# davidbau/rewriting

Hardware: AMD Instinct MI355X
Metric: images/sec StyleGANv2-1024 fwd (higher is better)
Workload: dtype f32 (conv operands split into exact f16 pairs from 32x32 up, f32 accumulate); 1 GPU; stylegan2-1024 generator forward (FFHQ-1024 architecture); batch_per_gpu=64, mconv=seq, weights=synthetic seed 0, parallelism=seeds partitioned per rank, no collective, matrix_mode=split, direct_sums=auto

## Files before the change

### include/rewriting_hip.h

```cpp
#ifndef REWRITING_HIP_H
#define REWRITING_HIP_H

#include <stdint.h>

#ifdef __cplusplus
extern "C" {
#endif

typedef void* rw_stream_t;

#define RW_ERR_BAD_ARGUMENT 10001
#define RW_ERR_UNSUPPORTED  10002

int rw_abi_version(void);
const char* rw_error_string(int code);


int rw_fused_bias_act_f32(const float* x, const float* b, const float* ref, float* y,
                          int64_t n, int64_t step_b, int64_t size_b,
                          int act, int grad, float alpha, float scale, rw_stream_t stream);
int rw_fused_bias_act_f16(const uint16_t* x, const uint16_t* b, const uint16_t* ref, uint16_t* y,
                          int64_t n, int64_t step_b, int64_t size_b,
                          int act, int grad, float alpha, float scale, rw_stream_t stream);
int rw_fused_bias_act_f64(const double* x, const double* b, const double* ref, double* y,
// ... 132 lines not shown
int rw_conv3x3_wino4h_to_rgb_f32(const float* x, const float* uf, int batch, int in_ch, int out_ch, int h, int w,
                                 float w_scale, const rw_conv_epilogue* ep, const rw_rgb_epilogue* rgb, float u_inv,
                                 const float* x_amax, rw_stream_t stream);
long long rw_packed_conv_transpose_blur_wino4h_elems(int out_ch, int in_ch);
int rw_pack_conv_transpose_blur_weight_wino4h_f32(const float* w, const float* k4, float* uf, int out_ch, int in_ch,
                                                  float u_scale, rw_stream_t stream);
int rw_conv_transpose3x3s2_blur_wino4h_f32(const float* x, const float* uf, float* y, int batch, int in_ch,
                                           int out_ch, int h, int w, float w_scale, const rw_conv_epilogue* ep,
                                           const float* post_scale, float u_inv, const float* x_amax,
                                           float* y_amax, rw_stream_t stream);

int rw_dconv3x3_supported(int out_ch, int in_ch, int h, int w);
long long rw_packed_dconv_weight_elems(int out_ch, int in_ch);
int rw_pack_dconv_weight_f32(const float* w, float* wp, int out_ch, int in_ch, float u_scale, rw_stream_t stream);
int rw_dconv3x3_f32(const float* x, const float* wp, float* y, int batch, int in_ch, int out_ch, int h, int w,
                    float w_scale, const rw_conv_epilogue* ep, float u_inv, const float* x_amax, float* y_amax,
                    rw_stream_t stream);
int rw_dconv3x3_rgb_partials(int out_ch);
int rw_dconv3x3_rgb_partial_f32(const float* x, const float* wp, float* y, int batch, int in_ch, int out_ch, int h, int w,
                                float w_scale, const rw_conv_epilogue* ep, const rw_rgb_epilogue* rgb, float u_inv,
                                const float* x_amax, float* y_amax, rw_stream_t stream);
int rw_rgb_combine_f32(const float* partials, int n_part, const float* bias, const float* skip, float* y, int batch,
                       int64_t hw, rw_stream_t stream);
int rw_dconv3x3_to_rgb_supported(int out_ch, int in_ch, int h, int w);
int rw_dconv3x3_to_rgb_f32(const float* x, const float* wp, int batch, int in_ch, int out_ch, int h, int w,
                           float w_scale, const rw_conv_epilogue* ep, const rw_rgb_epilogue* rgb, float u_inv,
                           const float* x_amax, rw_stream_t stream);
int rw_dconv_transpose_blur_supported(int out_ch, int in_ch, int h, int w);
long long rw_packed_dconv_transpose_blur_weight_elems(int out_ch, int in_ch);
int rw_pack_dconv_transpose_blur_weight_f32(const float* w, const float* k4, float* wp, int out_ch, int in_ch,
                                            float u_scale, rw_stream_t stream);
int rw_dconv_transpose3x3s2_blur_f32(const float* x, const float* wp, float* y, int batch, int in_ch, int out_ch, int h,
                                     int w, float w_scale, const rw_conv_epilogue* ep, const float* post_scale,
                                     float u_inv, const float* x_amax, float* y_amax, rw_stream_t stream);

int rw_tconv_blur_supported(int out_ch, int in_ch, int h, int w);
int rw_tconv_blur_f32(const float* x, const float* wp, const float* k4, float* y, int batch, int in_ch, int out_ch, int h,
                      int w, float w_scale, const rw_conv_epilogue* ep, const float* post_scale, float u_inv,
                      const float* x_amax, float* y_amax, rw_stream_t stream);

int rw_conv_transpose3x3s2_winoh_supported(int out_ch, int in_ch, int h, int w);
long long rw_packed_conv_transpose_winoh_elems(int out_ch, int in_ch);
int rw_pack_conv_transpose_winoh_f32(const float* w, float* uf, int out_ch, int in_ch, float u_scale, rw_stream_t stream);
int rw_conv_transpose3x3s2_winoh_f32(const float* x, const float* uf, float* y, int batch, int in_ch, int out_ch,
                                     int h, int w, float w_scale, const float* style, const float* demod, float u_inv,
                                     const float* x_amax, rw_stream_t stream);

int rw_noise_add_f32(const float* x, const float* noise, const float* noise_w, float* y,
                     int batch, int channels, int64_t hw, rw_stream_t stream);

int rw_blur_noise_act_f32(const float* x, const float* k4, const float* noise, const float* noise_w,
                          const float* bias, float* y, int batch, int channels, int out_h, int out_w,
                          rw_stream_t stream);
int rw_blur_noise_act_scaled_f32(const float* x, const float* k4, const float* noise, const float* noise_w,
                                 const float* bias, const float* post_scale, float* y, int batch, int channels,
                                 int out_h, int out_w, rw_stream_t stream);
int rw_blur_noise_act_amax_f32(const float* x, const float* k4, const float* noise, const float* noise_w,
                               const float* bias, const float* post_scale, float* y, int batch, int channels,
                               int out_h, int out_w, float* y_amax, rw_stream_t stream);

int rw_to_rgb_f32(const float* x, const float* w, const float* style, const float* bias,
                  const float* skip, float* y, int batch, int in_ch, int64_t hw, float w_scale,
                  rw_stream_t stream);


int64_t rw_second_moment_workspace_bytes(int channels, int64_t rows);
int rw_second_moment_f32(const float* a, float* mom2, int64_t rows, int channels, int64_t hw,
                         int layout, void* workspace, rw_stream_t stream);

int rw_channel_sums_f32(const float* a, float* sums, int64_t rows, int channels, int64_t hw,
                        int layout, int square_input, rw_stream_t stream);

#define RW_KEY_RESPONSE_MAX_KEYS 8
int rw_key_response_f32(const float* a, const float* keys, float* heat, float* peak,
                        int64_t images, int channels, int64_t hw, int n_keys, rw_stream_t stream);


typedef struct rw_solve_problem {
  int out_ch, in_ch, h, w, rank;
  const float* key;
  const float* style;
  const float* val;
  const float* bias;
  const float* noise;
  const float* noise_w;
  const float* context;
// ... 84 lines not shown
```

### rewriting_amd/_lib.py

```python
import ctypes
import os
from ctypes import (POINTER, Structure, c_char_p, c_double, c_float, c_int, c_int32, c_int64, c_uint,
                    c_void_p)

_HERE = os.path.dirname(os.path.abspath(__file__))
LIB_PATH = os.environ.get('RW_HIP_LIB') or os.path.join(_HERE, 'librewriting_hip.so')

ABI_VERSION = 10


class ConvEpilogue(Structure):
    _fields_ = [('style', c_void_p), ('demod', c_void_p), ('noise', c_void_p),
                ('noise_w', c_void_p), ('bias', c_void_p), ('act', c_int)]


class RgbEpilogue(Structure):
    _fields_ = [('weight', c_void_p), ('style', c_void_p), ('bias', c_void_p), ('skip', c_void_p),
                ('out', c_void_p), ('scale', c_float)]


class SolveProblem(Structure):
    _fields_ = [
        ('out_ch', c_int), ('in_ch', c_int), ('h', c_int), ('w', c_int), ('rank', c_int),
        ('key', c_void_p), ('style', c_void_p), ('val', c_void_p), ('bias', c_void_p),
# ... 93 lines not shown
    'rw_dconv_transpose_blur_weight_absmax_f32': (c_int, [c_void_p, c_void_p, c_int, c_int, c_void_p, c_void_p]),
    'rw_packed_conv_weight_wino4h_elems': (ctypes.c_longlong, [c_int, c_int]),
    'rw_pack_conv_weight_wino4h_f32': (c_int, [c_void_p, c_void_p, c_int, c_int, c_float, c_void_p]),
    'rw_conv3x3_wino4h_f32': (c_int, [c_void_p, c_void_p, c_void_p, c_int, c_int, c_int, c_int, c_int, c_float,
                                      POINTER(ConvEpilogue), c_float, c_void_p, c_void_p, c_void_p]),
    'rw_conv3x3_wino4h_to_rgb_f32': (c_int, [c_void_p, c_void_p, c_int, c_int, c_int, c_int, c_int, c_float,
                                             POINTER(ConvEpilogue), POINTER(RgbEpilogue), c_float, c_void_p, c_void_p]),
    'rw_packed_conv_transpose_blur_wino4h_elems': (ctypes.c_longlong, [c_int, c_int]),
    'rw_pack_conv_transpose_blur_weight_wino4h_f32': (c_int, [c_void_p, c_void_p, c_void_p, c_int, c_int, c_float,
                                                              c_void_p]),
    'rw_conv_transpose3x3s2_blur_wino4h_f32': (c_int, [c_void_p, c_void_p, c_void_p, c_int, c_int, c_int, c_int,
                                                       c_int, c_float, POINTER(ConvEpilogue), c_void_p, c_float,
                                                       c_void_p, c_void_p, c_void_p]),
    'rw_dconv3x3_supported': (c_int, [c_int, c_int, c_int, c_int]),
    'rw_packed_dconv_weight_elems': (ctypes.c_longlong, [c_int, c_int]),
    'rw_pack_dconv_weight_f32': (c_int, [c_void_p, c_void_p, c_int, c_int, c_float, c_void_p]),
    'rw_dconv3x3_f32': (c_int, [c_void_p, c_void_p, c_void_p, c_int, c_int, c_int, c_int, c_int, c_float,
                                POINTER(ConvEpilogue), c_float, c_void_p, c_void_p, c_void_p]),
    'rw_dconv3x3_rgb_partials': (c_int, [c_int]),
    'rw_dconv3x3_rgb_partial_f32': (c_int, [c_void_p, c_void_p, c_void_p, c_int, c_int, c_int, c_int, c_int, c_float,
                                            POINTER(ConvEpilogue), POINTER(RgbEpilogue), c_float, c_void_p, c_void_p,
                                            c_void_p]),
    'rw_rgb_combine_f32': (c_int, [c_void_p, c_int, c_void_p, c_void_p, c_void_p, c_int, c_int64, c_void_p]),
    'rw_dconv3x3_to_rgb_supported': (c_int, [c_int, c_int, c_int, c_int]),
    'rw_dconv3x3_to_rgb_f32': (c_int, [c_void_p, c_void_p, c_int, c_int, c_int, c_int, c_int, c_float,
                                       POINTER(ConvEpilogue), POINTER(RgbEpilogue), c_float, c_void_p, c_void_p]),
    'rw_dconv_transpose_blur_supported': (c_int, [c_int, c_int, c_int, c_int]),
    'rw_packed_dconv_transpose_blur_weight_elems': (ctypes.c_longlong, [c_int, c_int]),
    'rw_pack_dconv_transpose_blur_weight_f32': (c_int, [c_void_p, c_void_p, c_void_p, c_int, c_int, c_float, c_void_p]),
    'rw_dconv_transpose3x3s2_blur_f32': (c_int, [c_void_p, c_void_p, c_void_p, c_int, c_int, c_int, c_int, c_int,
                                                 c_float, POINTER(ConvEpilogue), c_void_p, c_float, c_void_p, c_void_p,
                                                 c_void_p]),
    'rw_tconv_blur_supported': (c_int, [c_int, c_int, c_int, c_int]),
    'rw_tconv_blur_f32': (c_int, [c_void_p, c_void_p, c_void_p, c_void_p, c_int, c_int, c_int, c_int, c_int, c_float,
                                  POINTER(ConvEpilogue), c_void_p, c_float, c_void_p, c_void_p, c_void_p]),
    'rw_conv_transpose_blur_wino4_supported': (c_int, [c_int, c_int, c_int, c_int]),
    'rw_packed_conv_transpose_blur_wino4_elems': (ctypes.c_longlong, [c_int, c_int]),
    'rw_pack_conv_transpose_blur_weight_wino4_f32': (c_int, [c_void_p, c_void_p, c_void_p, c_int, c_int, c_void_p]),
    'rw_conv_transpose3x3s2_blur_wino4_f32': (c_int, [c_void_p, c_void_p, c_void_p, c_int, c_int, c_int, c_int,
                                                      c_int, c_float, POINTER(ConvEpilogue), c_void_p, c_void_p]),
    'rw_blur_noise_act_scaled_f32': (c_int, [c_void_p, c_void_p, c_void_p, c_void_p, c_void_p, c_void_p, c_void_p,
                                             c_int, c_int, c_int, c_int, c_void_p]),
    'rw_blur_noise_act_amax_f32': (c_int, [c_void_p, c_void_p, c_void_p, c_void_p, c_void_p, c_void_p, c_void_p,
                                           c_int, c_int, c_int, c_int, c_void_p, c_void_p]),
    'rw_solve_ksplit': (c_int, [c_int, c_int, c_int, c_int]),
    'rw_solve_supported': (c_int, [c_int] * 7),
# ... 71 lines not shown
```

### rewriting_amd/csrc/rw_common.h

```cpp
#pragma once
#include <hip/hip_runtime.h>
#include <stdint.h>
#include <stdlib.h>
#include "../../include/rewriting_hip.h"

#define RW_WAVE 64

#define RW_CHECK_ARG(cond) do { if (!(cond)) return RW_ERR_BAD_ARGUMENT; } while (0)
#define RW_LAUNCH_RESULT() ((int)hipGetLastError())

static inline hipStream_t rw_s(rw_stream_t s) { return (hipStream_t)s; }

static inline int64_t rw_cdiv(int64_t a, int64_t b) { return (a + b - 1) / b; }

static inline int rw_cu_count(void) {
  static int cached[64];
  int dev = 0;
  if (hipGetDevice(&dev) != hipSuccess || dev < 0 || dev >= 64) return 256;
  if (cached[dev] == 0) {
    int n = 0;
    cached[dev] = (hipDeviceGetAttribute(&n, hipDeviceAttributeMultiprocessorCount, dev) == hipSuccess && n > 0) ? n : 256;
  }
  return cached[dev];
}
// ... 16 lines not shown
  for (int off = 32; off > 0; off >>= 1) v = fmaxf(v, __shfl_xor(v, off, 64));
  return v;
}

__device__ __forceinline__ float rw_block_sum_256(float v, float* lds4) {
  v = rw_wave_sum(v);
  const int wave = threadIdx.x >> 6;
  __syncthreads();
  if ((threadIdx.x & 63) == 0) lds4[wave] = v;
  __syncthreads();
  return lds4[0] + lds4[1] + lds4[2] + lds4[3];
}

typedef float rw_f32x16 __attribute__((ext_vector_type(16)));
typedef float rw_f32x4 __attribute__((ext_vector_type(4)));
typedef float rw_f32x2 __attribute__((ext_vector_type(2)));
typedef unsigned rw_u32x2 __attribute__((ext_vector_type(2)));
typedef unsigned rw_u32x4 __attribute__((ext_vector_type(4)));
typedef int rw_i32x4 __attribute__((ext_vector_type(4)));
typedef _Float16 rw_f16x2 __attribute__((ext_vector_type(2)));
typedef _Float16 rw_f16x4 __attribute__((ext_vector_type(4)));
typedef _Float16 rw_f16x8 __attribute__((ext_vector_type(8)));

template <int N> struct rw_int { static constexpr int value = N; };

__device__ __forceinline__ int rw_xcd_remap(int id, int total) {
  const int q = total >> 3, r = total & 7;
  const int xcd = id & 7, slot = id >> 3;
  const int base = (xcd < r) ? xcd * (q + 1) : r * (q + 1) + (xcd - r) * q;
  return base + slot;
}

__device__ __forceinline__ int rw_swz(int cc) { return (cc >> 1) & 3; }
__device__ __forceinline__ rw_f16x8 rw_expand(rw_f32x2 w) {
  const rw_f32x4 d = {w[0], w[1], w[0], w[1]};
  return __builtin_bit_cast(rw_f16x8, d);
}
__device__ __forceinline__ rw_f16x8 rw_pair(rw_f16x8 a, rw_f16x8 b) {
  return rw_f16x8{a[0], a[1], a[2], a[3], b[0], b[1], b[2], b[3]};
}
__device__ __forceinline__ rw_f16x8 rw_pair(rw_f32x2 a, rw_f32x2 b) {
  const rw_f32x4 d = {a[0], a[1], b[0], b[1]};
  return __builtin_bit_cast(rw_f16x8, d);
}

__device__ __forceinline__ void rw_dma_buffer_b32(unsigned lds_addr, int voffset, rw_i32x4 rsrc, int soffset) {
// ... 76 lines not shown
```

### rewriting_amd/csrc/rw_ops.hip

```cpp
#include "rw_common.h"
#ifndef OPS_NTS
#define OPS_NTS 0
#endif
#include <stdlib.h>
#include <stdint.h>

extern "C" int rw_abi_version(void) { return 10; }

extern "C" const char* rw_error_string(int code) {
  if (code == 0) return "success";
  if (code == RW_ERR_BAD_ARGUMENT) return "rewriting_hip: bad argument";
  if (code == RW_ERR_UNSUPPORTED) return "rewriting_hip: unsupported configuration";
  return hipGetErrorString((hipError_t)code);
}

template <typename T> struct RwAcc { typedef T type; };
template <> struct RwAcc<_Float16> { typedef float type; };

template <typename A>
__device__ __forceinline__ A rw_bias_act_one(A x, A ref, int code, A alpha, A scale) {
  A y;
  switch (code) {
    default:
    case 10: y = x; break;
// ... 957 lines not shown
    return rw_absmax_f32(y, (long long)n_out, y_amax, stream);
  }
  hipLaunchKernelGGL(blur_noise_act_kernel, dim3((unsigned)blocks), dim3(256), 0, rw_s(stream), x, k4,
                     noise, noise_w, bias, y, batch, channels, out_h, out_w, tiles_x, tiles_y, post_scale, y_amax);
  const int rc = RW_LAUNCH_RESULT();
  if (rc || !y_amax) return rc;
  return rw_bound_finish(y_amax, blocks, rw_s(stream));
}

extern "C" int rw_blur_noise_act_scaled_f32(const float* x, const float* k4, const float* noise,
                                            const float* noise_w, const float* bias, const float* post_scale,
                                            float* y, int batch, int channels, int out_h, int out_w,
                                            rw_stream_t stream) {
  return rw_blur_noise_act_amax_f32(x, k4, noise, noise_w, bias, post_scale, y, batch, channels, out_h, out_w, nullptr,
                                    stream);
}

extern "C" int rw_blur_noise_act_f32(const float* x, const float* k4, const float* noise,
                                     const float* noise_w, const float* bias, float* y, int batch,
                                     int channels, int out_h, int out_w, rw_stream_t stream) {
  return rw_blur_noise_act_scaled_f32(x, k4, noise, noise_w, bias, nullptr, y, batch, channels, out_h, out_w, stream);
}

__global__ void __launch_bounds__(256) to_rgb_kernel(const float* __restrict__ x,
                                                     const float* __restrict__ w,
                                                     const float* __restrict__ style,
                                                     const float* __restrict__ bias,
                                                     const float* __restrict__ skip,
                                                     float* __restrict__ y, int in_ch, int64_t hw,
                                                     float w_scale) {
  extern __shared__ float wm[];
  const int b = blockIdx.y;
  for (int t = threadIdx.x; t < 3 * in_ch; t += 256) {
    const int i = t % in_ch;
    wm[t] = w_scale * w[t] * style[(int64_t)b * in_ch + i];
  }
  __syncthreads();
  const int64_t hw4 = hw >> 2;
  const float* xb = x + (int64_t)b * in_ch * hw;
  for (int64_t q = (int64_t)blockIdx.x * 256 + threadIdx.x; q < hw4; q += (int64_t)gridDim.x * 256) {
    float4 a0 = make_float4(0.f, 0.f, 0.f, 0.f), a1 = a0, a2 = a0;
#pragma unroll 8
    for (int i = 0; i < in_ch; ++i) {
      const float4 v = reinterpret_cast<const float4*>(xb + (int64_t)i * hw)[q];
      const float w0 = wm[i], w1 = wm[in_ch + i], w2 = wm[2 * in_ch + i];
      a0.x += w0 * v.x; a0.y += w0 * v.y; a0.z += w0 * v.z; a0.w += w0 * v.w;
      a1.x += w1 * v.x; a1.y += w1 * v.y; a1.z += w1 * v.z; a1.w += w1 * v.w;
      a2.x += w2 * v.x; a2.y += w2 * v.y; a2.z += w2 * v.z; a2.w += w2 * v.w;
    }
    float4 acc[3] = {a0, a1, a2};
#pragma unroll
    for (int c = 0; c < 3; ++c) {
      const float bv = bias ? bias[c] : 0.f;
      float4 o = acc[c];
      o.x += bv; o.y += bv; o.z += bv; o.w += bv;
      const int64_t off = ((int64_t)b * 3 + c) * hw4 + q;
      if (skip) {
        const float4 s = reinterpret_cast<const float4*>(skip)[off];
        o.x += s.x; o.y += s.y; o.z += s.z; o.w += s.w;
      }
#if OPS_NTS & 2
      __builtin_nontemporal_store(rw_f32x4{o.x, o.y, o.z, o.w}, reinterpret_cast<rw_f32x4*>(y) + off);
#else
      reinterpret_cast<float4*>(y)[off] = o;
#endif
    }
  }
}

__global__ void __launch_bounds__(256) rgb_combine_kernel(const float* __restrict__ part, int n_part,
                                                          const float* __restrict__ bias, const float* __restrict__ skip,
                                                          float* __restrict__ y, int64_t n4, int64_t hw4, int64_t stride4) {
  for (int64_t q = (int64_t)blockIdx.x * 256 + threadIdx.x; q < n4; q += (int64_t)gridDim.x * 256) {
    float4 a = reinterpret_cast<const float4*>(part)[q];
    for (int k = 1; k < n_part; ++k) {
      const float4 v = reinterpret_cast<const float4*>(part)[q + k * stride4];
      a.x += v.x; a.y += v.y; a.z += v.z; a.w += v.w;
    }
    if (bias) {
      const float bv = bias[(q / hw4) % 3];
      a.x += bv; a.y += bv; a.z += bv; a.w += bv;
    }
    if (skip) {
      const float4 s = reinterpret_cast<const float4*>(skip)[q];
      a.x += s.x; a.y += s.y; a.z += s.z; a.w += s.w;
    }
    reinterpret_cast<float4*>(y)[q] = a;
  }
}

extern "C" int rw_rgb_combine_f32(const float* partials, int n_part, const float* bias, const float* skip, float* y,
                                  int batch, int64_t hw, rw_stream_t stream) {
  RW_CHECK_ARG(partials && y && n_part > 0 && batch > 0 && hw > 0);
  if (hw % 4) return RW_ERR_UNSUPPORTED;
  const int64_t n4 = (int64_t)batch * 3 * hw / 4;
  hipLaunchKernelGGL(rgb_combine_kernel, dim3(rw_stream_grid(n4, 256)), dim3(256), 0, rw_s(stream), partials, n_part, bias,
                     skip, y, n4, hw / 4, n4);
  return RW_LAUNCH_RESULT();
}

__global__ void __launch_bounds__(256) to_rgb_scalar_kernel(const float* __restrict__ x, const float* __restrict__ w,
                                                            const float* __restrict__ style,
                                                            const float* __restrict__ bias,
                                                            const float* __restrict__ skip, float* __restrict__ y,
                                                            int in_ch, int64_t hw, float w_scale) {
  extern __shared__ float wm[];
  const int b = blockIdx.y;
  for (int t = threadIdx.x; t < 3 * in_ch; t += 256) wm[t] = w_scale * w[t] * style[(int64_t)b * in_ch + t % in_ch];
  __syncthreads();
  const float* xb = x + (int64_t)b * in_ch * hw;
  for (int64_t q = (int64_t)blockIdx.x * 256 + threadIdx.x; q < hw; q += (int64_t)gridDim.x * 256) {
    float a[3] = {0.f, 0.f, 0.f};
    for (int i = 0; i < in_ch; ++i) {
      const float v = xb[(int64_t)i * hw + q];
      a[0] += wm[i] * v; a[1] += wm[in_ch + i] * v; a[2] += wm[2 * in_ch + i] * v;
    }
#pragma unroll
    for (int c = 0; c < 3; ++c) {
      const int64_t off = ((int64_t)b * 3 + c) * hw + q;
      float o = a[c] + (bias ? bias[c] : 0.f);
// ... 2 lines not shown
    }
  }
}

extern "C" int rw_to_rgb_f32(const float* x, const float* w, const float* style, const float* bias,
                             const float* skip, float* y, int batch, int in_ch, int64_t hw,
                             float w_scale, rw_stream_t stream) {
  RW_CHECK_ARG(x && w && style && y && batch > 0 && in_ch > 0 && hw > 0);
  if (hw % 4) {
    int gs = (int)rw_cdiv(hw, 256);
    if (gs > 2048) gs = 2048;
    hipLaunchKernelGGL(to_rgb_scalar_kernel, dim3(gs, batch), dim3(256), 3 * in_ch * sizeof(float), rw_s(stream), x, w,
                       style, bias, skip, y, in_ch, hw, w_scale);
    return RW_LAUNCH_RESULT();
  }
  int gx = (int)rw_cdiv(hw / 4, 256);
  const int cap = (256 * 8 + batch - 1) / batch;
  if (gx > cap) gx = cap;
  if (gx < 1) gx = 1;
  hipLaunchKernelGGL(to_rgb_kernel, dim3(gx, batch), dim3(256), 3 * in_ch * sizeof(float),
                     rw_s(stream), x, w, style, bias, skip, y, in_ch, hw, w_scale);
  return RW_LAUNCH_RESULT();
}
```

### rewriting_amd/hip.py

```python
import ctypes

import torch

from . import _lib
from ._lib import ConvEpilogue, RgbEpilogue, SolveProblem, check

SQRT2 = 2 ** 0.5


def _stream():
    return ctypes.c_void_p(torch.cuda.current_stream().cuda_stream)


def _dev(t, name='tensor', dtype=torch.float32):
    if not isinstance(t, torch.Tensor):
        raise TypeError('%s must be a torch.Tensor' % name)
    if not t.is_cuda:
        raise RuntimeError('rewriting_amd: %s is on %s; the HIP kernels need a GPU tensor '
                           '(there is no CPU fallback)' % (name, t.device))
    if t.dtype != dtype:
        if dtype == torch.float32:
            raise RuntimeError('rewriting_amd: %s is %s; the C ABI is fp32 only (RW_ERR_UNSUPPORTED, include/rewriting_hip.h: '
                               'the reference\'s pybind modules also dispatch half and double, this library does not) -- '
                               'cast the model / tensor with .float()' % (name, t.dtype))
# ... 163 lines not shown
def pack_conv_weight(weight, mode):
    weight = _dev(weight, 'weight')
    o, i = weight.shape[-4], weight.shape[-3]
    n = lib().rw_packed_conv_weight_elems(o, i, int(mode))
    if n <= 0:
        raise ValueError('bad weight shape / mode')
    wp = torch.empty(n, device=weight.device, dtype=weight.dtype)
    check(lib().rw_pack_conv_weight_f32(_p(weight), _p(wp), o, i, int(mode), _stream()))
    return wp


def _check_packed(wp, out_ch, in_ch, mode):
    if wp.numel() != lib().rw_packed_conv_weight_elems(out_ch, in_ch, mode):
        raise ValueError('packed weight does not come from pack_conv_weight(%d x %d, mode %d)'
                         % (out_ch, in_ch, mode))


def _epilogue(style=None, demod=None, noise=None, noise_w=None, bias=None, act=False):
    keep = [_opt(style, 'style'), _opt(demod, 'demod'), _opt(noise, 'noise'),
            _opt(noise_w, 'noise weight'), _opt(bias, 'bias')]
    ep = ConvEpilogue(_p(keep[0]).value, _p(keep[1]).value, _p(keep[2]).value,
                      _p(keep[3]).value, _p(keep[4]).value, int(bool(act)))
    return ep, keep


def _rgb_epilogue(rgb_weight, rgb_style, rgb_bias, rgb_skip, rgb_scale, out, x, out_ch):
    keep = [_dev(rgb_weight, 'rgb weight'), _dev(rgb_style, 'rgb style'), _opt(rgb_bias, 'rgb bias'),
            _opt(rgb_skip, 'rgb skip'), out]
    b, _, h, w = x.shape
    if tuple(keep[0].shape) != (3, out_ch) or tuple(keep[1].shape) != (b, out_ch):
        raise ValueError('rgb weight / style shapes')
    if keep[3] is not None and tuple(keep[3].shape) != (b, 3, h, w):
        raise ValueError('rgb skip shape')
    return RgbEpilogue(*[_p(t).value for t in keep], float(rgb_scale)), keep


def _packed(t, out_ch, in_ch, what, plain=None, split=None):
    wp = _dev(t, 'packed weight')
    if plain is not None and wp.numel() == plain(out_ch, in_ch):
        return wp, None
    if split is not None and wp.numel() == split(out_ch, in_ch):
        return wp, _u_inv(t)
    raise ValueError('packed weight does not come from %s(%d x %d)' % (what, out_ch, in_ch))


def _k4(k4):
# ... 376 lines not shown


def conv3x3_direct16_rgb_partial(x, wp, out_ch, w_scale, rgb_weight, rgb_style, rgb_scale, style=None, demod=None, noise=None,
                                 noise_w=None, bias=None, act=False, x_amax=None, y_amax=None):
    x = _dev(x, 'fmap')
    b, i, h, w = x.shape
    n_part = lib().rw_dconv3x3_rgb_partials(out_ch)
    if n_part <= 0:
        raise ValueError('no ToRGB partial sums for %d out-channels' % out_ch)
    part = torch.empty(n_part, b, 3, h, w, device=x.device, dtype=x.dtype)
    re, rgb_keep = _rgb_epilogue(rgb_weight, rgb_style, None, None, rgb_scale, part, x, out_ch)
    wp, u_inv = _packed(wp, out_ch, i, 'pack_conv_weight_direct16', split=lib().rw_packed_dconv_weight_elems)
    y = torch.empty(b, out_ch, h, w, device=x.device, dtype=x.dtype)
    ep, keep = _epilogue(style, demod, noise, noise_w, bias, act)
    x_amax, y_amax = _amax_in(x, x_amax), _amax_out(y_amax, y.numel())
    check(lib().rw_dconv3x3_rgb_partial_f32(_p(x), _p(wp), _p(y), b, i, out_ch, h, w, float(w_scale), ctypes.byref(ep),
                                            ctypes.byref(re), u_inv, _p(x_amax), _p(y_amax), _stream()))
    return y, part


def rgb_combine(partials, bias, skip):
    partials = _dev(partials, 'rgb partial sums')
    bias = _opt(bias, 'rgb bias')
    skip = _opt(skip, 'rgb skip')
    n, b, c, h, w = partials.shape
    if c != 3 or (skip is not None and tuple(skip.shape) != (b, 3, h, w)):
        raise ValueError('rgb partial / skip shapes')
    y = torch.empty(b, 3, h, w, device=partials.device, dtype=partials.dtype)
    check(lib().rw_rgb_combine_f32(_p(partials), n, _p(bias), _p(skip), _p(y), b, h * w, _stream()))
    return y


def conv3x3_direct16_to_rgb(x, wp, out_ch, w_scale, rgb_weight, rgb_style, rgb_bias, rgb_skip, rgb_scale, style=None,
                            demod=None, noise=None, noise_w=None, bias=None, act=False, x_amax=None):
    x = _dev(x, 'fmap')
    b, i, h, w = x.shape
    rgb = torch.empty(b, 3, h, w, device=x.device, dtype=x.dtype)
    re, rgb_keep = _rgb_epilogue(rgb_weight, rgb_style, rgb_bias, rgb_skip, rgb_scale, rgb, x, out_ch)
    wp, u_inv = _packed(wp, out_ch, i, 'pack_conv_weight_direct16', split=lib().rw_packed_dconv_weight_elems)
    ep, keep = _epilogue(style, demod, noise, noise_w, bias, act)
    x_amax = _amax_in(x, x_amax)
    check(lib().rw_dconv3x3_to_rgb_f32(_p(x), _p(wp), b, i, out_ch, h, w, float(w_scale), ctypes.byref(ep),
                                       ctypes.byref(re), u_inv, _p(x_amax), _stream()))
    return None, rgb


def pack_conv_transpose_blur_weight_direct16(weight, k4):
    weight = _dev(weight, 'weight')
    k4 = _k4(k4)
    o, i = weight.shape[-4], weight.shape[-3]
    n = lib().rw_packed_dconv_transpose_blur_weight_elems(o, i)
# ... 49 lines not shown
    return y


def blur_noise_act(x, k4, noise, noise_w, bias, post_scale=None, y_amax=None):
    x = _dev(x, 'fmap')
    k4 = _dev(k4, 'blur kernel')
    noise = _opt(noise, 'noise')
    noise_w = _opt(noise_w, 'noise weight')
    bias = _opt(bias, 'bias')
    b, c, ih, iw = x.shape
    y = torch.empty(b, c, ih - 1, iw - 1, device=x.device, dtype=x.dtype)
    post_scale = _post_scale(post_scale, b, c, 'channels')
    y_amax = _amax_out(y_amax, y.numel())
    check(lib().rw_blur_noise_act_amax_f32(_p(x), _p(k4), _p(noise), _p(noise_w), _p(bias), _p(post_scale), _p(y),
                                           b, c, ih - 1, iw - 1, _p(y_amax), _stream()))
    return y


def to_rgb(x, weight, style, bias, skip, w_scale):
    x = _dev(x, 'fmap')
    weight = _dev(weight, 'rgb weight')
    style = _dev(style, 'style')
    bias = _opt(bias, 'bias')
    skip = _opt(skip, 'skip')
    b, c, h, w = x.shape
    y = torch.empty(b, 3, h, w, device=x.device, dtype=x.dtype)
    check(lib().rw_to_rgb_f32(_p(x), _p(weight), _p(style), _p(bias), _p(skip), _p(y), b, c, h * w,
                              float(w_scale), _stream()))
    return y


_workspaces = {}


def _workspace(nbytes, device):
    key = (device.index, 'ws')
    ws = _workspaces.get(key)
    if ws is None or ws.numel() < nbytes:
        ws = torch.empty(max(nbytes, 1 << 20), dtype=torch.uint8, device=device)
        _workspaces[key] = ws
    return ws


def second_moment_accumulate(mom2, a, nchw=False):
    a = _dev(a, 'sample')
    if not (mom2.is_cuda and mom2.dtype == torch.float32 and mom2.is_contiguous()):
        raise RuntimeError('mom2 must be a contiguous float32 GPU tensor')
    if nchw:
        b, c, h, w = a.shape
# ... 296 lines not shown
```

### rewriting_amd/utils/stylegan2/models.py

```python
import contextlib
import math
import re
import threading
import warnings
from collections import OrderedDict, namedtuple

import numpy as np
import torch
from torch import nn

from . import grad, op, routing
from .routing import switches
from ... import hip


_weight_epoch = [0]


def bump_weight_epoch():
    _weight_epoch[0] += 1


class _DerivedWeights:

# ... 76 lines not shown
        if t is not None and t.dtype != x.dtype:
            raise RuntimeError('rewriting_amd: %s: the input is %s and the %s %s -- cast the model and its input to one '
                               'dtype, .float() or .double() (nothing is converted)' % (what, x.dtype, name, t.dtype))
    return True


def _forward_only_f64(what, *tensors):
    if torch.is_grad_enabled() and any(t is not None and t.requires_grad for t in tensors):
        raise NotImplementedError('rewriting_amd: %s: the float64 path is forward only -- no graph is recorded for double '
                                  'tensors (the adjoints in utils/stylegan2/grad.py are float32); run it under '
                                  'torch.no_grad(), or differentiate a .float() model' % what)


def _unhooked(*modules):
    return all('forward' not in m.__dict__ for m in modules)


def _idle():
    return dict(
        stream=None,
        aux=None,
        keep=[],
        final=None,
        image_path=False,
        switches=None,
        neighbours={},
        pre={},
        pre_join=None)


class _RunningForward(threading.local):
    def __init__(self):
        vars(self).update(_idle())


_running = _RunningForward()
_side_streams = {}
_Neighbours = namedtuple('_Neighbours', 'reader successor torgb')
_NO_NEIGHBOURS = _Neighbours(None, None, None)


class _scope:

    def __init__(self, **fields):
        self.fields = fields

# ... 6 lines not shown
        vars(_running).update(self.saved)


def _side_stream(device, which):
    stream = _side_streams.get((device, which))
    if stream is None:
        stream = _side_streams[device, which] = torch.cuda.Stream(device=device, priority=_switches().side_priority)
    return stream


@contextlib.contextmanager
def _side_streams_joined(device):
    main, side = torch.cuda.current_stream(), _side_stream(device, 'rgb')
    try:
        with _scope(stream=side, aux=_side_stream(device, 'aux')):
            yield main
    finally:
        main.wait_stream(side)
        del _running.keep[:]


def _rgb_stream():
    return _running.stream


def _prefetched(module):
    entry = _running.pre.get(id(module))
    if entry is not None and _running.pre_join is not None:
        torch.cuda.current_stream().wait_stream(_running.pre_join)
        _running.pre_join = None
    return entry


def _style_of(module, ahead, latent, index=None):
    styled = isinstance(module, StyledConvSeq)
    if ahead is not None:
        return ahead[0] if styled else ahead
    row = latent if index is None else latent[:, index]
    return module.mconv.modulation(DataBag(style=row)).style if styled else module.conv.modulation(row)


def _switches():
    return _running.switches or switches()


def fusion_enabled():
# ... 368 lines not shown
        super().__init__()
        self.factor = factor
        self.register_buffer('kernel', make_kernel(kernel) * (factor ** 2))
        p = self.kernel.shape[0] - factor
        self.pad = ((p + 1) // 2 + factor - 1, p // 2)

    def forward(self, input):
        return op.upfirdn2d(input, self.kernel, up=self.factor, down=1, pad=self.pad)


class UpsampleF(Upsample):
    def forward(self, d):
        return DataBag(d, fmap=super().forward(d.fmap))


class UpsampleO(Upsample):
    def __init__(self, kernel=[1, 3, 3, 1], factor=2):
        super().__init__(kernel, factor)

    def forward(self, d):
        side = _rgb_stream()
        if side is None:
            return DataBag(d, output=super().forward(d.output))
        with torch.cuda.stream(side):
            return DataBag(d, output=super().forward(d.output))


class NoiseInjectionF(nn.Module):
    def __init__(self):
        super().__init__()
        self.weight = nn.Parameter(torch.zeros(1))

    def noise_for(self, d, batch, height, width, device, double=False):
        noise = d.get('noise', None)
        if noise is None:
            rows = d.get('batch_rows', None)
            if rows is not None:
                start, total = rows
                return reference_noise(total, height * width, device, double)[start:start + batch]
            return reference_noise(batch, height * width, device, double)
        return noise.reshape(batch, height * width)

    def forward(self, d):
        b, _, h, w = d.fmap.shape
        if _double('NoiseInjectionF', d.fmap, weight=self.weight, noise=d.get('noise', None)):
            _forward_only_f64('NoiseInjectionF', d.fmap, self.weight)
            noise = self.noise_for(d, b, h, w, d.fmap.device, double=True)
            return DataBag(d, fmap=hip.noise_add_f64(d.fmap, noise, self.weight))
# ... 70 lines not shown

class ModulatedConv2dF(ModulatedConv2d):
    def forward(self, d):
        return DataBag(d, fmap=super().forward(d.fmap, d.style))


class ToRGBF(nn.Module):

    def __init__(self, in_channel, style_dim, upsample=True, blur_kernel=[1, 3, 3, 1], skip=False):
        super().__init__()
        if upsample:
            self.upsample = Upsample(blur_kernel)
        self.conv = ModulatedConv2d(in_channel, 3, 1, style_dim, demodulate=False)
        self.bias = nn.Parameter(torch.zeros(1, 3, 1, 1))
        self.skip = skip

    def forward(self, d):
        if d.get('fused_rgb') is not None:
            return DataBag(d, output=d.fused_rgb, fused_rgb=None)
        if _double('ToRGBF', d.fmap, weight=self.conv.weight, bias=self.bias, style=d.style,
                   skip=d.get('output') if self.skip else None):
            return self._forward_f64(d)
        skip = d.output if self.skip else None
        if skip is not None and tuple(skip.shape[2:]) != tuple(d.fmap.shape[2:]):
            up = self.upsample if hasattr(self, 'upsample') else Upsample([1, 3, 3, 1]).to(skip.device)
            if _rgb_stream() is None:
                skip = up(skip)
            else:
                with torch.cuda.stream(_rgb_stream()):
                    skip = up(skip)
        conv = self.conv
        side = _rgb_stream()
        partials = d.get('rgb_partials')
        if partials is not None:
            if side is None:
                raise RuntimeError('ToRGB partial sums outside the forward that produces them')
            side.wait_stream(torch.cuda.current_stream())
            with torch.cuda.stream(side):
                out = hip.rgb_combine(partials, self.bias.view(3), skip)
            _running.keep.append((partials,))
            nd = DataBag(d, output=out)
            nd.pop('rgb_partials', None)
            return nd
        if side is None:
            style = conv.modulation(d.style)
            weight, bias = conv.weight.view(3, conv.in_channel), self.bias.view(3)
            if grad.records(d.fmap, weight, style, bias, skip):
# ... 137 lines not shown
        nxt = _running.neighbours.get(id(self), _NO_NEIGHBOURS).successor
        if (nxt is not None and nxt[0]._fusable() and nxt[0]._standard_activation()
                and not nxt[0].mconv.upsample and nxt[0]._route(ctx, h, w).prescaled):
            post = _style_of(nxt[0], _prefetched(nxt[0]), d.latent, nxt[1])
        noise = self.noise.noise_for(d, fmap.shape[0], h, w, fmap.device)
        y_amax = self._result_bound(ctx, fmap, h, w)
        if route.runs_layer and not route.split:
            y_amax = None
        bound = dict(y_amax=y_amax) if y_amax is not None else {}
        if route.runs_layer:
            bound.update(dict(x_amax=x_amax) if route.split else {})
            out = dconv.run_whole_layer(fmap, style, route, fir, demod, noise=noise, post_scale=post, **bound,
                                        noise_w=self.noise.weight, bias=self.activate.bias, act=True)
        else:
            wide = dconv.run(fmap, style, style_on_load=True, demod=demod, x_amax=x_amax, route=route)
            out = hip.blur_noise_act(wide, fir, noise, self.noise.weight, self.activate.bias, post_scale=post, **bound)
        if y_amax is not None:
            out.rw_amax = (y_amax, out._version)
        return DataBag(d, style=style, fmap=out, **({} if post is None else dict(prescaled=post)))

    def _run_final(self, d, style, demod, x_amax, style_on_load, epilogue, route, received):
        _, torgb, idx = _running.final
        skip = d.output if torgb.skip else None
        if skip is not None and tuple(skip.shape[2:]) != tuple(d.fmap.shape[2:]):
            with _scope(final=None):
                return self.forward(received)
        main = torch.cuda.current_stream()
        if _running.stream is not None:
            main.wait_stream(_running.stream)
        rgb_style = _style_of(torgb, _prefetched(torgb), d.latent, idx)
        to_rgb = (torgb.conv.weight.view(3, torgb.conv.in_channel), rgb_style, torgb.bias.view(3), skip, torgb.conv.scale)
        _, rgb = self.mconv.dconv.run(d.fmap, style, style_on_load, demod=demod, x_amax=x_amax, to_rgb=to_rgb, route=route,
                                      **epilogue)
        return DataBag(d, style=style, fmap=None, fused_rgb=rgb)

    def _run_stride1(self, d, style, demod, ctx, x_amax, style_on_load, epilogue):
        fmap, (h, w) = d.fmap, d.fmap.shape[2:]
        route = self._route(ctx, h, w)
        y_amax = self._result_bound(ctx, fmap, h, w) if route.reports_bound else None
        tr = _running.neighbours.get(id(self), _NO_NEIGHBOURS).torgb if route.rgb_partials else None
        rgb = None
        if tr is not None:
            torgb, idx = tr
            rgb_style = _style_of(torgb, _prefetched(torgb), d.latent, idx)
            rgb = (torgb.conv.weight.view(3, torgb.conv.in_channel), rgb_style, torgb.conv.scale)
        out = self.mconv.dconv.run(fmap, style, style_on_load, demod=demod, x_amax=x_amax, y_amax=y_amax, rgb=rgb,
# ... 96 lines not shown
                     and not _running.image_path and _unhooked(*self.modules()))
            if not whole:
                return self._forward(input)
            topology = self._topology()
            with _scope(image_path=True, neighbours=topology[0]):
                return self._forward(input, topology)

    def _forward(self, input, topology=None):
        mb, from_res = micro_batch()
        micro = (mb and fusion_enabled() and torch.is_tensor(input) and not self.bag_output
                 and not self.bag_input and input.shape[0] > mb and 'up_rgb%d' % (int(math.log2(from_res)) - 2)
                 in self._modules and _running.stream is None and _unhooked(*self.modules()))
        side_ok = (not micro and fusion_enabled() and _switches().rgb_stream and torch.is_tensor(input)
                   and input.is_cuda and not self.bag_output and _running.stream is None
                   and not torch.cuda.is_current_stream_capturing()
                   and _unhooked(*self.modules()))
        if not micro and not side_ok:
            return super().forward(input)
        final = (topology or self._topology())[1] if _switches().fuse_final_rgb else None
        if micro:
            return self._forward_micro(input, mb, from_res, final)
        with contextlib.ExitStack() as scopes:
            main = scopes.enter_context(_side_streams_joined(input.device))
            scopes.enter_context(_scope(final=final))
            out = input
            for name, module in self._modules.items():
                out = module(out)
                if name == 'latents' and _running.image_path and _switches().prefetch_styles:
                    scopes.enter_context(_scope(**self._prefetch_modulations(out, _running.aux)))
        if torch.is_tensor(out):
            out.record_stream(main)
        return out

    def _forward_micro(self, z, mb, from_res, final):
        mods = list(self._modules.values())
        k = list(self._modules).index('up_rgb%d' % (int(math.log2(from_res)) - 2))
        d = z
        for m in mods[:k]:
            d = m(d)
        total = d.latent.shape[0]
        out = None
        with _scope(final=final):
            for s in range(0, total, mb):
                e = min(s + mb, total)
                part = DataBag({key: (v[s:e] if torch.is_tensor(v) and v.dim() > 0 and v.shape[0] == total else v)
                                for key, v in d.items()})
                part['batch_rows'] = (s, total)
                for m in mods[k:]:
                    part = m(part)
                if out is None:
                    out = part.new_empty((total,) + tuple(part.shape[1:]))
                out[s:e] = part
# ... 110 lines not shown
```

### rewriting_amd/utils/stylegan2/routing.py

```python
import os
from collections import namedtuple

from ... import hip

_CONV_IMPLS = {'auto': 0, 'mfma': 0, 'direct': 1, 'generic': 2, 'halo': 3, 'nosplitk': 5}
ONE_PASS_UP_MAX_IN = 64
FUSED_UP_MAX_IN = 512

Switches = namedtuple('Switches', [
    'fuse',
    'conv_impl',
    'conv_precision',
    'conv_algo',
    'up_algo',
    'mm',
    'mm_hooked_split',
    'mm_parts',
    'mm_direct16',
    'micro_batch',
    'up_fused',
    'up_fused2',
    'up_fused2_hooked',
    'up_fused2_max_in',
    'up_fused2_join',
    'direct16_small',
    'direct16_hooked',
    'dconv_ws_fwd',
    'dconv_v',
    'rgb_partial',
    'rgb_f4',
    'rgb_stream',
    'strip_stream',
    'side_priority',
    'prescale',
    'mm_no_handover',
    'prefetch_styles',
    'fuse_final_rgb',
])


def switches():
    env = os.environ.get
    direct16 = env('RW_MM_DIRECT16', 'auto')
    parts = env('RW_MM_PARTS')
    k, _, res = env('RW_MICRO_BATCH', '0').partition(':')
    return Switches(
        fuse=env('RW_FUSE', '1') != '0',
        conv_impl=_CONV_IMPLS[env('RW_CONV_IMPL', 'auto')],
        conv_precision=env('RW_CONV_PRECISION', 'f32'),
        conv_algo=env('RW_CONV_ALGO'),
        up_algo=env('RW_UP_ALGO', 'winograd'),
        mm=env('RW_MM'),
        mm_hooked_split=env('RW_MM_HOOKED', 'split') != 'f32',
        mm_parts=None if parts is None else tuple(parts.split(',')),
        mm_direct16={'auto': ('conv', 'up'), '1': ('conv', 'up', 'rgb')}.get(direct16) or tuple(direct16.split(',')),
        micro_batch=(int(k or 0), int(res or 256)),
        up_fused=env('RW_UP_FUSED', '1') != '0',
        up_fused2=env('RW_UP_FUSED2', '1') == '1',
        up_fused2_hooked=env('RW_UP_FUSED2_HOOKED', '1') == '1',
        up_fused2_max_in=int(env('RW_UP_FUSED2_MAX_IN', FUSED_UP_MAX_IN)),
        up_fused2_join=env('RW_UP_FUSED2_JOIN') == '1',
        direct16_small=env('RW_DIRECT16_SMALL', '1') != '0',
        direct16_hooked=env('RW_DIRECT16_HOOKED', '1') == '1',
        dconv_ws_fwd=env('RW_DCONV_WS_FWD', '1') != '0',
        dconv_v=env('RW_DCONV_V') == '1',
        rgb_partial=env('RW_RGB_PARTIAL', '1') != '0',
        rgb_f4=env('RW_RGB_F4', '1') != '0',
        rgb_stream=env('RW_RGB_STREAM', '1') != '0',
        strip_stream=env('RW_STRIP_STREAM', '1') != '0',
        side_priority=int(env('RW_SIDE_PRIORITY', '0')),
        prescale=env('RW_PRESCALE', '1') != '0',
        mm_no_handover=env('RW_MM_NO_HANDOVER') == '1',
        prefetch_styles=env('RW_PREFETCH_STYLES', '1') != '0',
        fuse_final_rgb=env('RW_FUSE_FINAL_RGB', '1') != '0',
    )


Context = namedtuple('Context', 'image_path on_device capturing rgb_stream aux_stream weight_changes')

STRIDE1_KERNELS = ('direct16', 'wino4_split', 'wino4', 'wino', 'bf16x6', 'gemm')
WHOLE_LAYER_KERNELS = ('fused', 'one_pass_direct16', 'one_pass_wino4')
UP_KERNELS = WHOLE_LAYER_KERNELS + ('f22_strips', 'halo_strips', 'plain')

Stride1Route = namedtuple('Stride1Route', 'kernel specialised rgb_partials reads_bound reports_bound prescaled')

UpRoute = namedtuple('UpRoute', 'kernel split side_strips reads_bound runs_layer')

FinalRgbRoute = namedtuple('FinalRgbRoute', 'kernel reads_bound')


# ... 111 lines not shown
```

Before: 1624 images/sec.

## Defer RGB skip upsampling and fuse it into to_rgb and partial combine

Instead of running a separate upfirdn2d upsample of the RGB skip image on the side stream, the upsample is marked as deferred and the 4-tap FIR upsample is computed inline when the next to_rgb or rgb partial-combine kernel reads the low-resolution skip. This removes one kernel launch and the full-resolution intermediate write and read per resolution. The cost is extra gather arithmetic inside the rgb kernels, plus version tracking to guard against in-place writes. The final layer's upsample stays eager, and any consumer that needs a real tensor materialises it.

```diff
diff --git a/include/rewriting_hip.h b/include/rewriting_hip.h
--- a/include/rewriting_hip.h
+++ b/include/rewriting_hip.h
@@ -178,6 +178,8 @@
                                 const float* x_amax, float* y_amax, rw_stream_t stream);
 int rw_rgb_combine_f32(const float* partials, int n_part, const float* bias, const float* skip, float* y, int batch,
                        int64_t hw, rw_stream_t stream);
+int rw_rgb_combine_up_f32(const float* partials, int n_part, const float* bias, const float* skip_lo, const float* fir,
+                          int pad0, int pad1, float* y, int batch, int h, int w, rw_stream_t stream);
 int rw_dconv3x3_to_rgb_supported(int out_ch, int in_ch, int h, int w);
 int rw_dconv3x3_to_rgb_f32(const float* x, const float* wp, int batch, int in_ch, int out_ch, int h, int w,
                            float w_scale, const rw_conv_epilogue* ep, const rw_rgb_epilogue* rgb, float u_inv,
@@ -218,6 +220,9 @@
 int rw_to_rgb_f32(const float* x, const float* w, const float* style, const float* bias,
                   const float* skip, float* y, int batch, int in_ch, int64_t hw, float w_scale,
                   rw_stream_t stream);
+int rw_to_rgb_up_f32(const float* x, const float* w, const float* style, const float* bias, const float* skip_lo,
+                     const float* fir, int pad0, int pad1, float* y, int batch, int in_ch, int h, int width,
+                     float w_scale, rw_stream_t stream);
 
 
 int64_t rw_second_moment_workspace_bytes(int channels, int64_t rows);
diff --git a/rewriting_amd/_lib.py b/rewriting_amd/_lib.py
--- a/rewriting_amd/_lib.py
+++ b/rewriting_amd/_lib.py
@@ -139,6 +139,10 @@
                                             POINTER(ConvEpilogue), POINTER(RgbEpilogue), c_float, c_void_p, c_void_p,
                                             c_void_p]),
     'rw_rgb_combine_f32': (c_int, [c_void_p, c_int, c_void_p, c_void_p, c_void_p, c_int, c_int64, c_void_p]),
+    'rw_rgb_combine_up_f32': (c_int, [c_void_p, c_int, c_void_p, c_void_p, c_void_p, c_int, c_int, c_void_p, c_int, c_int,
+                                      c_int, c_void_p]),
+    'rw_to_rgb_up_f32': (c_int, [c_void_p, c_void_p, c_void_p, c_void_p, c_void_p, c_void_p, c_int, c_int, c_void_p, c_int,
+                                 c_int, c_int, c_int, c_float, c_void_p]),
     'rw_dconv3x3_to_rgb_supported': (c_int, [c_int, c_int, c_int, c_int]),
     'rw_dconv3x3_to_rgb_f32': (c_int, [c_void_p, c_void_p, c_int, c_int, c_int, c_int, c_int, c_float,
                                        POINTER(ConvEpilogue), POINTER(RgbEpilogue), c_float, c_void_p, c_void_p]),
diff --git a/rewriting_amd/csrc/rw_common.h b/rewriting_amd/csrc/rw_common.h
--- a/rewriting_amd/csrc/rw_common.h
+++ b/rewriting_amd/csrc/rw_common.h
@@ -62,6 +62,50 @@
 typedef _Float16 rw_f16x4 __attribute__((ext_vector_type(4)));
 typedef _Float16 rw_f16x8 __attribute__((ext_vector_type(8)));
 
+template <int S>
+__device__ __forceinline__ void rw_up2k4_quad(const float* __restrict__ xm, int in_h, int in_w, int oy, int ox, int pad0,
+                                              const float* fir, float (&acc)[4]) {
+  const int cb = (ox + S - pad0) >> 1;
+  bool okc[4];
+  int cx[4];
+#pragma unroll
+  for (int d = 0; d < 4; ++d) {
+    okc[d] = (unsigned)(cb + d) < (unsigned)in_w;
+    cx[d] = min(max(cb + d, 0), in_w - 1);
+  }
+  const int a0 = (pad0 - oy) & 1;
+#pragma unroll
+  for (int j2 = 0; j2 < 2; ++j2) {
+    const int a = a0 + 2 * j2, vy = oy + a - pad0, iy = vy >> 1;
+    const bool okr = vy >= 0 && iy < in_h;
+    const float* xr = xm + (int64_t)min(max(iy, 0), in_h - 1) * in_w;
+    const float* kr = fir + 15 - 4 * a;
+    float col[4];
+#pragma unroll
+    for (int d = 0; d < 4; ++d) col[d] = xr[cx[d]];
+#pragma unroll
+    for (int e = 0; e < 4; ++e) {
+      const int c0 = (S + e) & 1;
+#pragma unroll
+      for (int j = 0; j < 2; ++j) {
+        const int d = ((e + c0 - S) >> 1) + j;
+        const float t = fmaf(col[d], kr[-(c0 + 2 * j)], acc[e]);
+        acc[e] = (okr && okc[d]) ? t : acc[e];
+      }
+    }
+  }
+}
+
+__device__ __forceinline__ void rw_up2k4_quad(const float* __restrict__ xm, int in_h, int in_w, int oy, int ox, int pad0,
+                                              const float* fir, float (&acc)[4]) {
+  if (pad0 & 1) rw_up2k4_quad<1>(xm, in_h, in_w, oy, ox, pad0, fir, acc);
+  else rw_up2k4_quad<0>(xm, in_h, in_w, oy, ox, pad0, fir, acc);
+}
+
+static inline bool rw_up2k4_ok(const float* skip_lo, const float* fir, int pad0, int pad1, int h, int w) {
+  return skip_lo && fir && pad0 >= 0 && pad1 >= 0 && pad0 + pad1 == 3 && h > 0 && w > 0 && h % 2 == 0 && w % 4 == 0;
+}
+
 template <int N> struct rw_int { static constexpr int value = N; };
 
 __device__ __forceinline__ int rw_xcd_remap(int id, int total) {
diff --git a/rewriting_amd/csrc/rw_ops.hip b/rewriting_amd/csrc/rw_ops.hip
--- a/rewriting_amd/csrc/rw_ops.hip
+++ b/rewriting_amd/csrc/rw_ops.hip
@@ -1003,15 +1003,14 @@
   return rw_blur_noise_act_scaled_f32(x, k4, noise, noise_w, bias, nullptr, y, batch, channels, out_h, out_w, stream);
 }
 
-__global__ void __launch_bounds__(256) to_rgb_kernel(const float* __restrict__ x,
-                                                     const float* __restrict__ w,
-                                                     const float* __restrict__ style,
-                                                     const float* __restrict__ bias,
-                                                     const float* __restrict__ skip,
-                                                     float* __restrict__ y, int in_ch, int64_t hw,
-                                                     float w_scale) {
+template <bool UP>
+__device__ __forceinline__ void to_rgb_body(const float* __restrict__ x, const float* __restrict__ w,
+                                            const float* __restrict__ style, const float* __restrict__ bias,
+                                            const float* __restrict__ skip, float* __restrict__ y, int in_ch, int64_t hw,
+                                            float w_scale, const float* __restrict__ fir, int pad0, int width) {
   extern __shared__ float wm[];
   const int b = blockIdx.y;
+  if (UP && threadIdx.x < 16) wm[3 * in_ch + threadIdx.x] = fir[threadIdx.x];
   for (int t = threadIdx.x; t < 3 * in_ch; t += 256) {
     const int i = t % in_ch;
     wm[t] = w_scale * w[t] * style[(int64_t)b * in_ch + i];
@@ -1030,13 +1029,19 @@
       a2.x += w2 * v.x; a2.y += w2 * v.y; a2.z += w2 * v.z; a2.w += w2 * v.w;
     }
     float4 acc[3] = {a0, a1, a2};
+    const int w4 = width >> 2, oy = UP ? (int)(q / w4) : 0, ox = UP ? ((int)q - oy * w4) * 4 : 0;
 #pragma unroll
     for (int c = 0; c < 3; ++c) {
       const float bv = bias ? bias[c] : 0.f;
       float4 o = acc[c];
       o.x += bv; o.y += bv; o.z += bv; o.w += bv;
       const int64_t off = ((int64_t)b * 3 + c) * hw4 + q;
-      if (skip) {
+      if (UP) {
+        float s[4] = {0.f, 0.f, 0.f, 0.f};
+        rw_up2k4_quad(skip + ((int64_t)b * 3 + c) * hw4, (int)(hw4 / (width >> 1)), width >> 1, oy, ox, pad0,
+                      wm + 3 * in_ch, s);
+        o.x += s[0]; o.y += s[1]; o.z += s[2]; o.w += s[3];
+      } else if (skip) {
         const float4 s = reinterpret_cast<const float4*>(skip)[off];
         o.x += s.x; o.y += s.y; o.z += s.z; o.w += s.w;
       }
@@ -1049,6 +1054,24 @@
   }
 }
 
+__global__ void __launch_bounds__(256) to_rgb_kernel(const float* __restrict__ x,
+                                                     const float* __restrict__ w,
+                                                     const float* __restrict__ style,
+                                                     const float* __restrict__ bias,
+                                                     const float* __restrict__ skip,
+                                                     float* __restrict__ y, int in_ch, int64_t hw,
+                                                     float w_scale) {
+  to_rgb_body<false>(x, w, style, bias, skip, y, in_ch, hw, w_scale, nullptr, 0, 0);
+}
+
+__global__ void __launch_bounds__(256) to_rgb_up_kernel(const float* __restrict__ x, const float* __restrict__ w,
+                                                        const float* __restrict__ style, const float* __restrict__ bias,
+                                                        const float* __restrict__ skip_lo, const float* __restrict__ fir,
+                                                        int pad0, float* __restrict__ y, int in_ch, int64_t hw, int width,
+                                                        float w_scale) {
+  to_rgb_body<true>(x, w, style, bias, skip_lo, y, in_ch, hw, w_scale, fir, pad0, width);
+}
+
 __global__ void __launch_bounds__(256) rgb_combine_kernel(const float* __restrict__ part, int n_part,
                                                           const float* __restrict__ bias, const float* __restrict__ skip,
                                                           float* __restrict__ y, int64_t n4, int64_t hw4, int64_t stride4) {
@@ -1077,6 +1100,47 @@
   const int64_t n4 = (int64_t)batch * 3 * hw / 4;
   hipLaunchKernelGGL(rgb_combine_kernel, dim3(rw_stream_grid(n4, 256)), dim3(256), 0, rw_s(stream), partials, n_part, bias,
                      skip, y, n4, hw / 4, n4);
+  return RW_LAUNCH_RESULT();
+}
+
+__global__ void __launch_bounds__(256) rgb_combine_up_kernel(const float* __restrict__ part, int n_part,
+                                                             const float* __restrict__ bias,
+                                                             const float* __restrict__ skip_lo,
+                                                             const float* __restrict__ fir, int pad0,
+                                                             float* __restrict__ y, int64_t n4, int h, int w,
+                                                             int64_t stride4) {
+  __shared__ float sk[16];
+  if (threadIdx.x < 16) sk[threadIdx.x] = fir[threadIdx.x];
+  __syncthreads();
+  const int w4 = w >> 2, in_h = h >> 1, in_w = w >> 1;
+  const int64_t hw4 = (int64_t)h * w4;
+  for (int64_t q = (int64_t)blockIdx.x * 256 + threadIdx.x; q < n4; q += (int64_t)gridDim.x * 256) {
+    float4 a = reinterpret_cast<const float4*>(part)[q];
+    for (int k = 1; k < n_part; ++k) {
+      const float4 v = reinterpret_cast<const float4*>(part)[q + k * stride4];
+      a.x += v.x; a.y += v.y; a.z += v.z; a.w += v.w;
+    }
+    const int64_t plane = q / hw4;
+    if (bias) {
+      const float bv = bias[plane % 3];
+      a.x += bv; a.y += bv; a.z += bv; a.w += bv;
+    }
+    const int r = (int)(q - plane * hw4), oy = r / w4, ox = (r - oy * w4) * 4;
+    float s[4] = {0.f, 0.f, 0.f, 0.f};
+    rw_up2k4_quad(skip_lo + plane * in_h * in_w, in_h, in_w, oy, ox, pad0, sk, s);
+    a.x += s[0]; a.y += s[1]; a.z += s[2]; a.w += s[3];
+    reinterpret_cast<float4*>(y)[q] = a;
+  }
+}
+
+extern "C" int rw_rgb_combine_up_f32(const float* partials, int n_part, const float* bias, const float* skip_lo,
+                                     const float* fir, int pad0, int pad1, float* y, int batch, int h, int w,
+                                     rw_stream_t stream) {
+  RW_CHECK_ARG(partials && y && skip_lo && fir && n_part > 0 && batch > 0 && h > 0 && w > 0);
+  if (!rw_up2k4_ok(skip_lo, fir, pad0, pad1, h, w)) return RW_ERR_UNSUPPORTED;
+  const int64_t n4 = (int64_t)batch * 3 * h * (w / 4);
+  hipLaunchKernelGGL(rgb_combine_up_kernel, dim3(rw_stream_grid(n4, 256)), dim3(256), 0, rw_s(stream), partials, n_part,
+                     bias, skip_lo, fir, pad0, y, n4, h, w, n4);
   return RW_LAUNCH_RESULT();
 }
 
@@ -1125,3 +1189,18 @@
                      rw_s(stream), x, w, style, bias, skip, y, in_ch, hw, w_scale);
   return RW_LAUNCH_RESULT();
 }
+
+extern "C" int rw_to_rgb_up_f32(const float* x, const float* w, const float* style, const float* bias,
+                                const float* skip_lo, const float* fir, int pad0, int pad1, float* y, int batch,
+                                int in_ch, int h, int width, float w_scale, rw_stream_t stream) {
+  RW_CHECK_ARG(x && w && style && y && skip_lo && fir && batch > 0 && in_ch > 0 && h > 0 && width > 0);
+  if (!rw_up2k4_ok(skip_lo, fir, pad0, pad1, h, width)) return RW_ERR_UNSUPPORTED;
+  const int64_t hw = (int64_t)h * width;
+  int gx = (int)rw_cdiv(hw / 4, 256);
+  const int cap = (256 * 8 + batch - 1) / batch;
+  if (gx > cap) gx = cap;
+  if (gx < 1) gx = 1;
+  hipLaunchKernelGGL(to_rgb_up_kernel, dim3(gx, batch), dim3(256), (3 * in_ch + 16) * sizeof(float), rw_s(stream), x, w,
+                     style, bias, skip_lo, fir, pad0, y, in_ch, hw, width, w_scale);
+  return RW_LAUNCH_RESULT();
+}
diff --git a/rewriting_amd/hip.py b/rewriting_amd/hip.py
--- a/rewriting_amd/hip.py
+++ b/rewriting_amd/hip.py
@@ -209,6 +209,37 @@
     ep = ConvEpilogue(_p(keep[0]).value, _p(keep[1]).value, _p(keep[2]).value,
                       _p(keep[3]).value, _p(keep[4]).value, int(bool(act)))
     return ep, keep
+
+
+def defer_up(image, fir, pad):
+    fir = _k4(fir)
+    pad = (int(pad[0]), int(pad[1]))
+    if sum(pad) != 3 or min(pad) < 0:
+        raise ValueError('an upsampling is deferred only where the image doubles exactly (pads that sum to 3)')
+    image.rw_up = (fir, pad, image._version)
+    return image
+
+
+def deferred_up(image):
+    mark = getattr(image, 'rw_up', None)
+    if mark is None:
+        return None
+    fir, pad, version = mark
+    if version != image._version:
+        raise RuntimeError('rewriting_amd: a running image whose upsampling was deferred has been written in place')
+    return fir, pad
+
+
+def _skip_lo(skip, b, h, w):
+    mark = None if skip is None else deferred_up(skip)
+    skip = _opt(skip, 'rgb skip')
+    if mark is None:
+        if skip is not None and tuple(skip.shape) != (b, 3, h, w):
+            raise ValueError('rgb skip shape')
+        return skip, None
+    if tuple(skip.shape) != (b, 3, h // 2, w // 2) or h % 2 or w % 4:
+        raise ValueError('deferred rgb skip shape')
+    return skip, (mark[0], mark[1][0], mark[1][1])
 
 
 def _rgb_epilogue(rgb_weight, rgb_style, rgb_bias, rgb_skip, rgb_scale, out, x, out_ch):
@@ -631,11 +662,15 @@
 def rgb_combine(partials, bias, skip):
     partials = _dev(partials, 'rgb partial sums')
     bias = _opt(bias, 'rgb bias')
-    skip = _opt(skip, 'rgb skip')
     n, b, c, h, w = partials.shape
-    if c != 3 or (skip is not None and tuple(skip.shape) != (b, 3, h, w)):
+    if c != 3:
         raise ValueError('rgb partial / skip shapes')
+    skip, up = _skip_lo(skip, b, h, w)
     y = torch.empty(b, 3, h, w, device=partials.device, dtype=partials.dtype)
+    if up is not None:
+        check(lib().rw_rgb_combine_up_f32(_p(partials), n, _p(bias), _p(skip), _p(up[0]), up[1], up[2], _p(y), b, h, w,
+                                          _stream()))
+        return y
     check(lib().rw_rgb_combine_f32(_p(partials), n, _p(bias), _p(skip), _p(y), b, h * w, _stream()))
     return y
 
@@ -731,9 +766,14 @@
     weight = _dev(weight, 'rgb weight')
     style = _dev(style, 'style')
     bias = _opt(bias, 'bias')
+    b, c, h, w = x.shape
+    up = None if skip is None or deferred_up(skip) is None else _skip_lo(skip, b, h, w)[1]
     skip = _opt(skip, 'skip')
-    b, c, h, w = x.shape
     y = torch.empty(b, 3, h, w, device=x.device, dtype=x.dtype)
+    if up is not None:
+        check(lib().rw_to_rgb_up_f32(_p(x), _p(weight), _p(style), _p(bias), _p(skip), _p(up[0]), up[1], up[2], _p(y), b, c,
+                                     h, w, float(w_scale), _stream()))
+        return y
     check(lib().rw_to_rgb_f32(_p(x), _p(weight), _p(style), _p(bias), _p(skip), _p(y), b, c, h * w,
                               float(w_scale), _stream()))
     return y
diff --git a/rewriting_amd/utils/stylegan2/models.py b/rewriting_amd/utils/stylegan2/models.py
--- a/rewriting_amd/utils/stylegan2/models.py
+++ b/rewriting_amd/utils/stylegan2/models.py
@@ -122,6 +122,7 @@
         aux=None,
         keep=[],
         final=None,
+        eager_up=None,
         image_path=False,
         switches=None,
         neighbours={},
@@ -174,6 +175,20 @@
 
 def _rgb_stream():
     return _running.stream
+
+
+def _materialised(image):
+    if not torch.is_tensor(image) or hip.deferred_up(image) is None:
+        return image
+    fir, pad = hip.deferred_up(image)
+    side = _rgb_stream()
+    with contextlib.nullcontext() if side is None else torch.cuda.stream(side):
+        return op.upfirdn2d(image.detach(), fir, up=2, down=1, pad=pad)
+
+
+def _skip_inline(skip, fmap):
+    return (skip is not None and hip.deferred_up(skip) is not None and fmap.shape[3] % 4 == 0
+            and tuple(fmap.shape[2:]) == (2 * skip.shape[2], 2 * skip.shape[3]))
 
 
 def _prefetched(module):
@@ -588,8 +603,16 @@
         side = _rgb_stream()
         if side is None:
             return DataBag(d, output=super().forward(d.output))
+        image = d.output
+        if (_running.image_path and _switches().rgb_inline_up and torch.is_tensor(image) and image.is_cuda
+                and image.dtype is torch.float32 and image.dim() == 4 and image.shape[3] % 2 == 0 and self.factor == 2
+                and tuple(self.kernel.shape) == (4, 4) and sum(self.pad) == 3 and hip.deferred_up(image) is None
+                and _running.eager_up is not self):
+            low = hip.defer_up(image.detach(), self.kernel, self.pad)
+            _running.keep.append((image,))
+            return DataBag(d, output=low)
         with torch.cuda.stream(side):
-            return DataBag(d, output=super().forward(d.output))
+            return DataBag(d, output=super().forward(_materialised(image)))
 
 
 class NoiseInjectionF(nn.Module):
@@ -706,7 +729,9 @@
                    skip=d.get('output') if self.skip else None):
             return self._forward_f64(d)
         skip = d.output if self.skip else None
-        if skip is not None and tuple(skip.shape[2:]) != tuple(d.fmap.shape[2:]):
+        if _rgb_stream() is None or not _skip_inline(skip, d.fmap):
+            skip = _materialised(skip)
+        if skip is not None and hip.deferred_up(skip) is None and tuple(skip.shape[2:]) != tuple(d.fmap.shape[2:]):
             up = self.upsample if hasattr(self, 'upsample') else Upsample([1, 3, 3, 1]).to(skip.device)
             if _rgb_stream() is None:
                 skip = up(skip)
@@ -890,6 +915,7 @@
     def _run_final(self, d, style, demod, x_amax, style_on_load, epilogue, route, received):
         _, torgb, idx = _running.final
         skip = d.output if torgb.skip else None
+        skip = _materialised(skip)
         if skip is not None and tuple(skip.shape[2:]) != tuple(d.fmap.shape[2:]):
             with _scope(final=None):
                 return self.forward(received)
@@ -1032,12 +1058,14 @@
             return self._forward_micro(input, mb, from_res, final)
         with contextlib.ExitStack() as scopes:
             main = scopes.enter_context(_side_streams_joined(input.device))
-            scopes.enter_context(_scope(final=final))
+            ups = [m for m in self._modules.values() if isinstance(m, UpsampleO)]
+            scopes.enter_context(_scope(final=final, eager_up=ups[-1] if final is not None and ups else None))
             out = input
             for name, module in self._modules.items():
                 out = module(out)
                 if name == 'latents' and _running.image_path and _switches().prefetch_styles:
                     scopes.enter_context(_scope(**self._prefetch_modulations(out, _running.aux)))
+        out = _materialised(out)
         if torch.is_tensor(out):
             out.record_stream(main)
         return out
diff --git a/rewriting_amd/utils/stylegan2/routing.py b/rewriting_amd/utils/stylegan2/routing.py
--- a/rewriting_amd/utils/stylegan2/routing.py
+++ b/rewriting_amd/utils/stylegan2/routing.py
@@ -29,6 +29,7 @@
     'dconv_v',
     'rgb_partial',
     'rgb_f4',
+    'rgb_inline_up',
     'rgb_stream',
     'strip_stream',
     'side_priority',
@@ -66,6 +67,7 @@
         dconv_v=env('RW_DCONV_V') == '1',
         rgb_partial=env('RW_RGB_PARTIAL', '1') != '0',
         rgb_f4=env('RW_RGB_F4', '1') != '0',
+        rgb_inline_up=env('RW_RGB_INLINE_UP', '1') != '0',
         rgb_stream=env('RW_RGB_STREAM', '1') != '0',
         strip_stream=env('RW_STRIP_STREAM', '1') != '0',
         side_priority=int(env('RW_SIDE_PRIORITY', '0')),
```

New measurement: 1622 images/sec. About the same (-0.1%).
